# teamtomo/torch-motion-correction

Hardware: NVIDIA B200
Metric: movies_per_second_estimate_plus_correct (higher is better)
Workload: dtype f32

## Files before the change

torch_motion_correction_b200/csrc/optimizer_tiled.cu:

```cuda
#include "common.cuh"
#include <math.h>

namespace {

constexpr int kTileKy = 8, kTileKx = 16, kTileBins = kTileKy * kTileKx;
#ifndef TMC_CHUNK_FRAMES
#define TMC_CHUNK_FRAMES 8
#endif
constexpr int kChunkFrames = TMC_CHUNK_FRAMES;
constexpr int kMaxChunks = 256 / kChunkFrames;
constexpr int kTileThreads = 256;
constexpr int kCoefThreads = 1024;

struct StepParams {
  const float* spec;
  const int* tiles;
  int n_tiles, G, T;
  int ny, nx, KY, KX, ky_start;
  float inv_ny, inv_nx;
  const double* sum_norms;
  const float* eval_base;
  const float* w_t;
  const float* w_sp;
  int nt, nhw;
  const float* patch_scale;
  float pixel_spacing;
  int loss_type;
  float* coef;
  float* exp_avg;
  float* exp_avg_sq;
  float step_size, bc2_sqrt, w1, w2, b2, epsf, weight_decay;
  double* loss_out;
  float* grad_out;
  float* shifts;
  float* grad_shifts;
  double* q;
};

__device__ __forceinline__ uint32_t smem_u32(const void* p) { return (uint32_t)__cvta_generic_to_shared(p); }
__device__ __forceinline__ void mbar_init(uint64_t* bar, int count) {
  asm volatile("mbarrier.init.shared::cta.b64 [%0], %1;" ::"r"(smem_u32(bar)), "r"(count));
}
__device__ __forceinline__ void mbar_expect_tx(uint64_t* bar, uint32_t bytes) {
  asm volatile("mbarrier.arrive.expect_tx.shared::cta.b64 _, [%0], %1;" ::"r"(smem_u32(bar)), "r"(bytes) : "memory");
}
__device__ __forceinline__ void bulk_load(void* dst, const void* src, uint32_t bytes, uint64_t* bar) {
  asm volatile("cp.async.bulk.shared::cluster.global.mbarrier::complete_tx::bytes [%0], [%1], %2, [%3];" ::"r"(smem_u32(dst)),
               "l"(src), "r"(bytes), "r"(smem_u32(bar))
               : "memory");
}
__device__ __forceinline__ void mbar_wait_addr(uint32_t bar_addr, uint32_t parity) {
  asm volatile(
      "{\n"
      ".reg .pred P1;\n"
      "LAB_WAIT:\n"
      "mbarrier.try_wait.parity.shared::cta.b64 P1, [%0], %1;\n"
      "@P1 bra DONE;\n"
      "bra LAB_WAIT;\n"
      "DONE:\n"
      "}" ::"r"(bar_addr),
      "r"(parity)
      : "memory");
}
__device__ __forceinline__ void mbar_wait(uint64_t* bar, uint32_t parity) {
  asm volatile(
      "{\n"
      ".reg .pred P1;\n"
      "LAB_WAIT:\n"
      "mbarrier.try_wait.parity.shared::cta.b64 P1, [%0], %1;\n"
      "@P1 bra DONE;\n"
      "bra LAB_WAIT;\n"
      "DONE:\n"
      "}" ::"r"(smem_u32(bar)),
      "r"(parity)
      : "memory");
}

__device__ __forceinline__ float2 fast_cis(float x) {
  const float k = rintf(x * 0.15915494309189535f);
  float r = fmaf(k, -6.2831854820251465f, x);
  r = fmaf(k, 1.7484555e-7f, r);
  return make_float2(__cosf(r), __sinf(r));
}

__global__ void __launch_bounds__(kCoefThreads) local_coefficient_kernel(const StepParams p, int flags) {
  extern __shared__ float csm[];
  __shared__ double red[kCoefThreads / 32];
  const int tid = threadIdx.x;
  const int G = p.G, T = p.T, nt = p.nt, nhw = p.nhw;
  const int ncoef = 2 * nt * nhw, ngt = 2 * G * T;
  float* gs_s = csm;
  float* eb_s = gs_s + ngt;
  float* wt_s = eb_s + ngt;
  float* wsp_s = wt_s + T * nt;
  float* coef_s = wsp_s + G * nhw;
  float* u_s = coef_s + ncoef;
  float* ea_s = u_s + G * 2 * nt;
  float* eas_s = ea_s + ncoef;
  asm volatile("griddepcontrol.launch_dependents;");
  const float neg_inv_px = -1.0f / p.pixel_spacing;
  if (flags & 4)
    for (int i = tid; i < ngt; i += kCoefThreads) eb_s[i] = __ldg(p.eval_base + i);
  for (int i = tid; i < T * nt; i += kCoefThreads) wt_s[i] = __ldg(p.w_t + i);
  for (int i = tid; i < G * nhw; i += kCoefThreads) wsp_s[i] = __ldg(p.w_sp + i);
  asm volatile("griddepcontrol.wait;" ::: "memory");
  if (flags & 1)
    for (int i = tid; i < ngt; i += kCoefThreads) gs_s[i] = p.grad_shifts[i] * neg_inv_px;
  for (int i = tid; i < ncoef; i += kCoefThreads) coef_s[i] = p.coef[i];
  if (flags & (2 | 8))
    for (int i = tid; i < ncoef; i += kCoefThreads) {
      ea_s[i] = p.exp_avg[i];
      eas_s[i] = p.exp_avg_sq[i];
    }
  double l = 0.0;
  if (flags & 1) {
    for (int g = tid; g < G; g += kCoefThreads) {
      const double sc = (double)p.patch_scale[g];
      if (sc != 0.0) {
        const double sumA = p.sum_norms[g], qg = p.q[g];
        if (p.loss_type == 0) {
          const double a = (double)T / (double)(T - 1);
          l += sc * a * a * (sumA - qg / T);
        } else {
          l += -sc * (qg - sumA) / ((double)p.ny * (double)p.nx * (double)(T - 1));
        }
      }
    }
    l = warp_sum(l);
    if ((tid & 31) == 0) red[tid >> 5] = l;
  }
  __syncthreads();
  if (flags & 1) {
    if (tid == 0) {
      double s = 0.0;
      for (int i = 0; i < kCoefThreads / 32; ++i) s += red[i];
      *p.loss_out = s;
    }
    for (int i = tid; i < ngt; i += kCoefThreads) p.grad_shifts[i] = 0.f;
    for (int i = tid; i < G; i += kCoefThreads) p.q[i] = 0.0;
    for (int o = tid; o < G * 2 * nt; o += kCoefThreads) {
      const int k = o % nt, c = (o / nt) & 1, g = o / (2 * nt);
      float acc = 0.f;
      for (int t = 0; t < T; ++t) acc = fmaf(wt_s[t * nt + k], gs_s[(g * T + t) * 2 + c], acc);
      u_s[o] = acc;
    }
    __syncthreads();
    const float step_size = p.step_size, bc2_sqrt = p.bc2_sqrt, w1 = p.w1, w2 = p.w2, b2 = p.b2, epsf = p.epsf;
    for (int o = tid; o < ncoef; o += kCoefThreads) {
      const int j = o % nhw, ck = o / nhw;
      float acc = 0.f;
      for (int g = 0; g < G; ++g) acc = fmaf(wsp_s[g * nhw + j], u_s[g * 2 * nt + ck], acc);
      p.grad_out[o] = acc;
      if (flags & 2) {
        float gr = acc;
        float par = coef_s[o];
        if (p.weight_decay != 0.f) gr = __fadd_rn(gr, __fmul_rn(p.weight_decay, par));
        const float m = __fadd_rn(ea_s[o], __fmul_rn(w1, __fsub_rn(gr, ea_s[o])));
        const float v = __fadd_rn(__fmul_rn(eas_s[o], b2), __fmul_rn(w2, __fmul_rn(gr, gr)));
        p.exp_avg[o] = m;
        p.exp_avg_sq[o] = v;
        const float denom = __fadd_rn(__fdiv_rn(__fsqrt_rn(v), bc2_sqrt), epsf);
        par = __fadd_rn(par, __fmul_rn(-step_size, __fdiv_rn(m, denom)));
        p.coef[o] = par;
        coef_s[o] = par;
      }
    }
    __syncthreads();
  }
  if (flags & 8) {
    const float step_size = p.step_size, bc2_sqrt = p.bc2_sqrt, w1 = p.w1, w2 = p.w2, b2 = p.b2, epsf = p.epsf;
    for (int o = tid; o < ncoef; o += kCoefThreads) {
      float gr = p.grad_out[o];
      float par = coef_s[o];
      if (p.weight_decay != 0.f) gr = __fadd_rn(gr, __fmul_rn(p.weight_decay, par));
      const float m = __fadd_rn(ea_s[o], __fmul_rn(w1, __fsub_rn(gr, ea_s[o])));
      const float v = __fadd_rn(__fmul_rn(eas_s[o], b2), __fmul_rn(w2, __fmul_rn(gr, gr)));
      p.exp_avg[o] = m;
      p.exp_avg_sq[o] = v;
      const float denom = __fadd_rn(__fdiv_rn(__fsqrt_rn(v), bc2_sqrt), epsf);
      par = __fadd_rn(par, __fmul_rn(-step_size, __fdiv_rn(m, denom)));
      p.coef[o] = par;
      coef_s[o] = par;
    }
    __syncthreads();
  }
  if (!(flags & 4)) return;
  for (int o = tid; o < G * 2 * nt; o += kCoefThreads) {
    const int ck = o % (2 * nt), g = o / (2 * nt);
    float acc = 0.f;
    for (int j = 0; j < nhw; ++j) acc = fmaf(wsp_s[g * nhw + j], coef_s[ck * nhw + j], acc);
    u_s[o] = acc;
  }
  __syncthreads();
  for (int i = tid; i < ngt; i += kCoefThreads) {
    const int c = i & 1, t = (i >> 1) % T, g = (i >> 1) / T;
    float ev = 0.f;
    for (int k = 0; k < nt; ++k) ev = fmaf(wt_s[t * nt + k], u_s[(g * 2 + c) * nt + k], ev);
    const float v = __fmul_rn(-1.0f, __fadd_rn(ev, eb_s[(t * G + g) * 2 + c]));
    p.shifts[i] = __fdiv_rn(v, p.pixel_spacing);
  }
}

__global__ void __launch_bounds__(kTileThreads) local_loss_tile_kernel(const StepParams p) {
  constexpr int THREADS = kTileThreads;
  constexpr int NW = THREADS / 64;
  extern __shared__ __align__(128) unsigned char smem_raw[];
  const int T = p.T;
  float* tile = reinterpret_cast<float*>(smem_raw);
  float4* Ey = reinterpret_cast<float4*>(tile + (long)T * 256);
  float4* Ex = Ey + T * 8;
  float4* Cy = Ex + T * 8;
  float4* Cx = Cy + 64;
  float* sigma = reinterpret_cast<float*>(Cx + 64);
  float* cf = sigma + 256;
  double* red = reinterpret_cast<double*>(cf + 24);
  uint64_t* bars = reinterpret_cast<uint64_t*>(red + 2);

  const int tid = threadIdx.x;
  const int g = blockIdx.y, tile_id = blockIdx.x;
  const int nchunks = (T + kChunkFrames - 1) / kChunkFrames;
  asm volatile("griddepcontrol.launch_dependents;");

  if (tid == 0) {
    for (int c = 0; c < nchunks; ++c) mbar_init(bars + c, 1);
    asm volatile("fence.mbarrier_init.release.cluster;" ::: "memory");
    asm volatile("fence.proxy.async.shared::cta;" ::: "memory");
    const float* src = p.spec + ((long)g * p.n_tiles + tile_id) * T * 256;
    for (int c = 0; c < nchunks; ++c) {
      const int frames = min(kChunkFrames, T - c * kChunkFrames);
      const uint32_t bytes = (uint32_t)frames * 256 * sizeof(float);
      mbar_expect_tx(bars + c, bytes);
      bulk_load(tile + (long)c * kChunkFrames * 256, src + (long)c * kChunkFrames * 256, bytes, bars + c);
    }
  }
  const float sc = __ldg(p.patch_scale + g);
  const int ty = __ldg(p.tiles + 2 * tile_id), tx = __ldg(p.tiles + 2 * tile_id + 1);
  constexpr int kRowThreads = 96;
  const int my_r = tid < kRowThreads ? (tid & 7) : kTileKy + ((tid - kRowThreads) & 15);
  float my_cf;
  {
    if (my_r < kTileKy) {
      int ky = p.ky_start + min(ty * kTileKy + my_r, p.KY - 1);
      if (ky >= (p.ny + 1) / 2) ky -= p.ny;
      if (ky < -(p.ny / 2)) ky += p.ny;
      my_cf = __fmul_rn(-6.283185307179586f, __fmul_rn((float)ky, p.inv_ny));
    } else {
      my_cf = __fmul_rn(-6.283185307179586f, __fmul_rn((float)min(tx * kTileKx + my_r - kTileKy, p.KX - 1), p.inv_nx));
    }
    if (tid < kTileKy) cf[tid] = my_cf;
    if (tid >= kRowThreads && tid < kRowThreads + kTileKx) cf[kTileKy + tid - kRowThreads] = my_cf;
  }
  sigma[tid] = 0.f;
  asm volatile("griddepcontrol.wait;" ::: "memory");
  if (sc == 0.f || T < 2) {
    __syncthreads();
    for (int c = 0; c < nchunks; ++c) mbar_wait(bars + c, 0);
    return;
  }
  const float* shg = p.shifts + (long)g * T * 2;
  if (tid < kRowThreads) {
    for (int t = tid >> 3; t < T; t += kRowThreads / 8) {
      const float2 e = fast_cis(__fmul_rn(my_cf, shg[2 * t]));
      Ey[t * 8 + my_r] = make_float4(e.x, e.x, e.y, e.y);
    }
  } else {
    const int j = (tid - kRowThreads) & 15;
    for (int t = (tid - kRowThreads) >> 4; t < T; t += (kTileThreads - kRowThreads) / 16) {
      const float2 e = fast_cis(__fmul_rn(my_cf, shg[2 * t + 1]));
      float* o = reinterpret_cast<float*>(Ex + t * 8 + (j >> 1)) + (j & 1);
      o[0] = e.x;
      o[2] = e.y;
    }
  }
  __syncthreads();

  {
    const int pb = tid & 63, th = tid >> 6;
    const float4* ey = Ey + (pb >> 3) + th * 8;
    const float4* ex = Ex + (pb & 7) + th * 8;
    float2* col = reinterpret_cast<float2*>(tile) + pb + th * 128;
    float2 sre = make_float2(0.f, 0.f), sim = make_float2(0.f, 0.f);
    auto body = [&](const float4* eyp, const float4* exp_, float2* cp) {
      const float4 y = *eyp, x = *exp_;
      const float2 cy = make_float2(y.x, y.y), sy = make_float2(y.z, y.w);
      const float2 cx = make_float2(x.x, x.y), sx = make_float2(x.z, x.w);
      const float2 ere = __ffma2_rn(make_float2(-sy.x, -sy.y), sx, __fmul2_rn(cy, cx));
      const float2 eim = __ffma2_rn(sy, cx, __fmul2_rn(cy, sx));
      const float2 a = cp[0], b = cp[64];
      const float2 re = __ffma2_rn(make_float2(-b.x, -b.y), eim, __fmul2_rn(a, ere));
      const float2 im = __ffma2_rn(b, ere, __fmul2_rn(a, eim));
      cp[0] = re;
      cp[64] = im;
      sre = __fadd2_rn(sre, re);
      sim = __fadd2_rn(sim, im);
    };
    const uint32_t bar0 = smem_u32(bars);
    for (int c = 0; c < nchunks; ++c) {
      mbar_wait_addr(bar0 + 8u * c, 0);
      if ((c + 1) * kChunkFrames <= T) {
#pragma unroll
        for (int i = 0; i < kChunkFrames / NW; ++i) body(ey + i * NW * 8, ex + i * NW * 8, col + i * NW * 128);
      } else {
        for (int t = c * kChunkFrames + th, i = 0; t < T; t += NW, ++i) body(ey + i * NW * 8, ex + i * NW * 8, col + i * NW * 128);
      }
      ey += kChunkFrames * 8;
      ex += kChunkFrames * 8;
      col += kChunkFrames * 128;
    }
    atomicAdd(sigma + pb, sre.x);
    atomicAdd(sigma + 64 + pb, sre.y);
    atomicAdd(sigma + 128 + pb, sim.x);
    atomicAdd(sigma + 192 + pb, sim.y);
  }
  __syncthreads();
  if (tid < 64) {
    const int pb = tid;
    const float2 re = make_float2(sigma[pb], sigma[64 + pb]), im = make_float2(sigma[128 + pb], sigma[192 + pb]);
    const int kx0 = tx * kTileKx + 2 * (pb & 7);
    const float w0 = (p.loss_type == 0 || kx0 == 0 || 2 * kx0 == p.nx) ? 1.0f : 2.0f;
    const float w1 = (p.loss_type == 0 || 2 * (kx0 + 1) == p.nx) ? 1.0f : 2.0f;
    const float cfy = cf[pb >> 3], cfx0 = cf[8 + 2 * (pb & 7)], cfx1 = cf[9 + 2 * (pb & 7)];
    const float wr0 = w0 * re.x, wr1 = w1 * re.y, wi0 = w0 * im.x, wi1 = w1 * im.y;
    Cy[pb] = make_float4(cfy * wr0, cfy * wr1, -cfy * wi0, -cfy * wi1);
    Cx[pb] = make_float4(cfx0 * wr0, cfx1 * wr1, -cfx0 * wi0, -cfx1 * wi1);
  }
  __syncthreads();

  float bscale;
  if (p.loss_type == 0) {
    const float a = (float)T / (float)(T - 1);
    bscale = -sc * a * a / (float)T;
  } else {
    bscale = -sc / ((float)p.ny * (float)p.nx * (float)(T - 1));
  }
  const int lane = tid & 31, warp = tid >> 5;
  const int half = lane >> 4, l16 = lane & 15;
  for (int pi = warp; 2 * pi < T; pi += THREADS / 32) {
    const int t = 2 * pi + half;
    const bool ok = t < T;
    const float2* row = reinterpret_cast<const float2*>(tile + (long)(ok ? t : 0) * 256) + l16;
    float2 ay = make_float2(0.f, 0.f), ax = make_float2(0.f, 0.f);
#pragma unroll
    for (int k = 0; k < 4; ++k) {
      const float2 re = row[16 * k], im = row[64 + 16 * k];
      const float4 cy = Cy[l16 + 16 * k], cx = Cx[l16 + 16 * k];
      ay = __ffma2_rn(im, make_float2(cy.x, cy.y), ay);
      ay = __ffma2_rn(re, make_float2(cy.z, cy.w), ay);
      ax = __ffma2_rn(im, make_float2(cx.x, cx.y), ax);
      ax = __ffma2_rn(re, make_float2(cx.z, cx.w), ax);
    }
    const float gy = ay.x + ay.y, gx = ax.x + ax.y;
    const bool keep_x = (l16 & 8) != 0;
    float v = (keep_x ? gx : gy) + __shfl_xor_sync(0xffffffffu, keep_x ? gy : gx, 8);
#pragma unroll
    for (int o = 4; o > 0; o >>= 1) v += __shfl_xor_sync(0xffffffffu, v, o);
    if (ok && (l16 & 7) == 0) {
      v *= -2.0f * bscale;
      if (v != 0.f) atomicAdd(p.grad_shifts + ((long)g * T + t) * 2 + (keep_x ? 1 : 0), v);
    }
  }
  if (tid < 64) {
    const int pb = tid;
    const float2 re = make_float2(sigma[pb], sigma[64 + pb]), im = make_float2(sigma[128 + pb], sigma[192 + pb]);
    const int kx0 = tx * kTileKx + 2 * (pb & 7);
    const float w0 = (p.loss_type == 0 || kx0 == 0 || 2 * kx0 == p.nx) ? 1.0f : 2.0f;
    const float w1 = (p.loss_type == 0 || 2 * (kx0 + 1) == p.nx) ? 1.0f : 2.0f;
    double v = (double)w0 * ((double)re.x * re.x + (double)im.x * im.x) + (double)w1 * ((double)re.y * re.y + (double)im.y * im.y);
    v = warp_sum(v);
    if ((tid & 31) == 0 && v != 0.0) atomicAdd(p.q + g, v);
  }
}

__global__ void tile_spectra_kernel(const float2* __restrict__ spec, int T, int Tp, int KY, int KX, const int* __restrict__ tiles,
                                    int n_tiles, int frame_major, float* __restrict__ out) {
  const int tile_id = blockIdx.x, t = blockIdx.y, g = blockIdx.z, G = gridDim.z;
  const int b = threadIdx.x;
  const int kyb = tiles[2 * tile_id] * kTileKy + b / kTileKx, kx = tiles[2 * tile_id + 1] * kTileKx + b % kTileKx;
  float2 v = make_float2(0.f, 0.f);
  const long plane = frame_major ? ((long)(t >> 1) * G + g) * 2 + (t & 1) : (long)g * Tp + t;
  if (kyb < KY && kx < KX) v = spec[(plane * KY + kyb) * KX + kx];
  float* o = out + (((long)g * n_tiles + tile_id) * T + t) * 2 * kTileBins;
  o[b] = v.x;
  o[kTileBins + b] = v.y;
}

size_t tile_smem_bytes(int t) {
  return (size_t)t * kTileBins * 8 + (size_t)t * 16 * 16 + 128 * 16 + 256 * 4 + 24 * 4 + 2 * 8 +
         (size_t)((t + kChunkFrames - 1) / kChunkFrames) * 8;
}
size_t coef_smem_bytes(int g, int t, int nt, int nhw) {
  return ((size_t)4 * g * t + (size_t)t * nt + (size_t)g * nhw + (size_t)6 * nt * nhw + (size_t)g * 2 * nt) * 4;
}

}

TMC_API int tmc_local_steps_supported(int g, int t, int nt, int nhw) {
  if (t < 2 || t > kChunkFrames * kMaxChunks || g < 1 || g > 65535 || nt < 1 || nhw < 1) return 0;
  if (tile_smem_bytes(t) > 200 * 1024) return 0;
  return coef_smem_bytes(g, t, nt, nhw) <= 160 * 1024 ? 1 : 0;
}

TMC_API int tmc_local_tile_spectra(const void* spec, int g, int t, int tp, int ky_count, int kx_count, const int* tiles,
                                   int n_tiles, int frame_major, void* out, cudaStream_t stream) {
  TMC_CHECK_ARG(spec && tiles && out && g >= 1 && t >= 1 && tp >= t && n_tiles >= 1 && t <= 65535 && g <= 65535,
                "local_tile_spectra: bad arguments");
  dim3 grid(n_tiles, t, g);
  tile_spectra_kernel<<<grid, kTileBins, 0, stream>>>((const float2*)spec, t, tp, ky_count, kx_count, tiles, n_tiles, frame_major, (float*)out);
  tmc_count_launch();
  TMC_CHECK_LAUNCH("tmc_local_tile_spectra");
  return TMC_OK;
}

TMC_API long tmc_local_steps_workspace_bytes(int g, int t, int nt) {
  (void)nt;
  long floats = 4l * g * t;
  floats = (floats + 1) & ~1l;
  return floats * 4 + 8l * g;
}

TMC_API int tmc_local_steps(const void* tiled, const int* tiles, int n_tiles, int g, int t, int ny, int nx, int ky_count,
                            int kx_count, int ky_start, const double* sum_norms, const float* eval_base, const float* w_t,
                            const float* w_sp, int nt, int nhw, const float* patch_scale, float pixel_spacing, int loss_type,
                            float* coef, float* exp_avg, float* exp_avg_sq, double lr, double beta1, double beta2, double eps,
                            double weight_decay, int first_row, int mode, int n_steps, double* loss_out, float* grad_out,
                            void* workspace, cudaStream_t stream) {
  TMC_CHECK_ARG(tiled && tiles && sum_norms && eval_base && w_t && w_sp && patch_scale && coef && loss_out && grad_out && workspace,
                "local_steps: null pointer");
  TMC_CHECK_ARG(mode >= 0 && mode <= 3, "local_steps: mode must be 0 .. 3");
  TMC_CHECK_ARG(mode == 1 || (exp_avg && exp_avg_sq), "local_steps: Adam state missing");
  TMC_CHECK_ARG(mode == 0 || n_steps == 1, "local_steps: modes 1 .. 3 take one step");
  TMC_CHECK_ARG(n_tiles >= 1 && n_steps >= 1 && first_row >= 0 && pixel_spacing > 0.f && (loss_type == 0 || loss_type == 1),
                "local_steps: bad arguments");
  if (!tmc_local_steps_supported(g, t, nt, nhw)) {
    tmc_set_error("local_steps: unsupported problem size (g=%d t=%d nt=%d nhw=%d)", g, t, nt, nhw);
    return TMC_ERR_UNSUPPORTED;
  }
  StepParams p;
  p.spec = (const float*)tiled;
  p.tiles = tiles;
  p.n_tiles = n_tiles;
  p.G = g;
  p.T = t;
  p.ny = ny;
  p.nx = nx;
  p.KY = ky_count;
  p.KX = kx_count;
  p.ky_start = ky_start;
  p.inv_ny = (float)(1.0 / (double)ny);
  p.inv_nx = (float)(1.0 / (double)nx);
  p.sum_norms = sum_norms;
  p.eval_base = eval_base;
  p.w_t = w_t;
  p.w_sp = w_sp;
  p.nt = nt;
  p.nhw = nhw;
  p.pixel_spacing = pixel_spacing;
  p.loss_type = loss_type;
  p.coef = coef;
  p.exp_avg = exp_avg;
  p.exp_avg_sq = exp_avg_sq;
  p.w1 = (float)(1.0 - beta1);
  p.w2 = (float)(1.0 - beta2);
  p.b2 = (float)beta2;
  p.epsf = (float)eps;
  p.weight_decay = (float)weight_decay;
  p.step_size = 0.f;
  p.bc2_sqrt = 1.f;
  p.grad_out = grad_out;
  float* wf = (float*)workspace;
  p.shifts = wf;
  p.grad_shifts = wf + 2l * g * t;
  const long floats = (4l * g * t + 1) & ~1l;
  p.q = (double*)(wf + floats);
  if (mode < 2) TMC_CUDA(cudaMemsetAsync(workspace, 0, (size_t)tmc_local_steps_workspace_bytes(g, t, nt), stream));
  const size_t smem = tile_smem_bytes(t), csmem = coef_smem_bytes(g, t, nt, nhw);
  TMC_CUDA(cudaFuncSetAttribute(local_loss_tile_kernel, cudaFuncAttributeMaxDynamicSharedMemorySize, (int)(200 * 1024)));
  TMC_CUDA(cudaFuncSetAttribute(local_coefficient_kernel, cudaFuncAttributeMaxDynamicSharedMemorySize, (int)(160 * 1024)));
  dim3 grid(n_tiles, g);
  p.patch_scale = patch_scale + (long)first_row * g;
  p.loss_out = loss_out;
  if (mode >= 2) {
    const double step = (double)first_row;
    p.step_size = (float)(lr / (1.0 - pow(beta1, step)));
    p.bc2_sqrt = (float)sqrt(1.0 - pow(beta2, step));
  }
  local_coefficient_kernel<<<1, kCoefThreads, csmem, stream>>>(p, mode == 2 ? (8 | 4) : (mode == 3 ? 8 : 4));
  tmc_count_launch();
  if (mode == 3) {
    TMC_CHECK_LAUNCH("tmc_local_steps");
    return TMC_OK;
  }
  cudaLaunchAttribute attr[1];
  attr[0].id = cudaLaunchAttributeProgrammaticStreamSerialization;
  attr[0].val.programmaticStreamSerializationAllowed = 1;
  cudaLaunchConfig_t cfg = {};
  cfg.gridDim = grid;
  cfg.blockDim = dim3(kTileThreads);
  cfg.dynamicSmemBytes = smem;
  cfg.stream = stream;
  cfg.attrs = attr;
  cfg.numAttrs = 1;
  cudaLaunchConfig_t ccfg = {};
  ccfg.gridDim = dim3(1);
  ccfg.blockDim = dim3(kCoefThreads);
  ccfg.dynamicSmemBytes = csmem;
  ccfg.stream = stream;
  ccfg.attrs = attr;
  ccfg.numAttrs = 1;
  for (int i = 0; i < n_steps; ++i) {
    const int row = first_row + i;
    p.patch_scale = patch_scale + (long)row * g;
    const double step = (double)(row + 1);
    p.step_size = (float)(lr / (1.0 - pow(beta1, step)));
    p.bc2_sqrt = (float)sqrt(1.0 - pow(beta2, step));
    p.loss_out = loss_out + (mode == 0 ? row : 0);
    TMC_CUDA(cudaLaunchKernelEx(&cfg, local_loss_tile_kernel, p));
    tmc_count_launch();
    const int last = i == n_steps - 1;
    TMC_CUDA(cudaLaunchKernelEx(&ccfg, local_coefficient_kernel, p, mode == 0 ? (last ? 3 : 7) : 1));
    tmc_count_launch();
  }
  TMC_CHECK_LAUNCH("tmc_local_steps");
  return TMC_OK;
}
```

Baseline: 51.65.

## Add persistent register-resident tiled loss kernel with double-buffered bulk loads

Adds a templated loss kernel for short frame counts (up to 64) that keeps each tile's spectra in registers, runs as a persistent grid sized to the occupancy limit, and double-buffers tile loads with TMA bulk copies and mbarriers. Per-frame gradient sums use a shuffle transpose-reduce instead of shared-memory reductions, and the arithmetic uses packed float2 math. The old shared-memory kernel stays as the fallback for larger T. Risks are higher register pressure and lower occupancy.

```diff
diff --git a/torch_motion_correction_b200/csrc/optimizer_tiled.cu b/torch_motion_correction_b200/csrc/optimizer_tiled.cu
--- a/torch_motion_correction_b200/csrc/optimizer_tiled.cu
+++ b/torch_motion_correction_b200/csrc/optimizer_tiled.cu
@@ -1,5 +1,7 @@
 #include "common.cuh"
 #include <math.h>
+
+#include <algorithm>
 
 namespace {
 
@@ -11,6 +13,8 @@
 constexpr int kMaxChunks = 256 / kChunkFrames;
 constexpr int kTileThreads = 256;
 constexpr int kCoefThreads = 1024;
+constexpr int kRegWarps = kTileThreads / 32;
+constexpr int kRegMaxFrames = 8;
 
 struct StepParams {
   const float* spec;
@@ -98,6 +102,9 @@
   float* ea_s = u_s + G * 2 * nt;
   float* eas_s = ea_s + ncoef;
   asm volatile("griddepcontrol.launch_dependents;");
+#ifdef TMC_COEF_NOOP
+  return;
+#endif
   const float neg_inv_px = -1.0f / p.pixel_spacing;
   if (flags & 4)
     for (int i = tid; i < ngt; i += kCoefThreads) eb_s[i] = __ldg(p.eval_base + i);
@@ -201,7 +208,243 @@
   }
 }
 
+__device__ __forceinline__ float tile_freq(const StepParams& p, int ty, int tx, int r) {
+  if (r < kTileKy) {
+    int ky = p.ky_start + min(ty * kTileKy + r, p.KY - 1);
+    if (ky >= (p.ny + 1) / 2) ky -= p.ny;
+    if (ky < -(p.ny / 2)) ky += p.ny;
+    return __fmul_rn(-6.283185307179586f, __fmul_rn((float)ky, p.inv_ny));
+  }
+  return __fmul_rn(-6.283185307179586f, __fmul_rn((float)min(tx * kTileKx + r - kTileKy, p.KX - 1), p.inv_nx));
+}
+
+template <int N, int O>
+__device__ __forceinline__ float transpose_reduce(const float (&v)[N], int lane, int& idx, int& live) {
+  if constexpr (N == 1) {
+    float s = v[0];
+#pragma unroll
+    for (int o = O; o > 0; o >>= 1) s += __shfl_xor_sync(0xffffffffu, s, o);
+    if (O > 0 && (lane & (2 * O - 1)) != 0) live = 0;
+    return s;
+  } else {
+    static_assert(O > 0, "more values than lanes");
+    constexpr int H = (N + 1) / 2;
+    const bool up = (lane & O) != 0;
+    float w[H];
+#pragma unroll
+    for (int i = 0; i < H; ++i) {
+      const float lo = v[i], hi = i + H < N ? v[i + H] : 0.f;
+      w[i] = (up ? hi : lo) + __shfl_xor_sync(0xffffffffu, up ? lo : hi, O);
+    }
+    if (up) {
+      idx += H;
+      live -= H;
+    } else {
+      live = min(live, H);
+    }
+    return transpose_reduce<H, O / 2>(w, lane, idx, live);
+  }
+}
+
+template <int NF>
 __global__ void __launch_bounds__(kTileThreads) local_loss_tile_kernel(const StepParams p) {
+  constexpr int TF = NF * kRegWarps;
+  extern __shared__ __align__(128) float4 ring[];
+  __shared__ float2 ey_s[TF][kTileKy];
+  __shared__ float4 exc_s[TF][kTileKx / 4];
+  __shared__ float4 exs_s[TF][kTileKx / 4];
+  __shared__ float4 part_s[kRegWarps][2][32];
+  __shared__ __align__(16) float sig_s[2 * kTileBins];
+  __shared__ __align__(16) float cf_s[kTileKy + kTileKx];
+  __shared__ uint64_t bars[2];
+
+  const int tid = threadIdx.x, lane = tid & 31, warp = tid >> 5;
+  const int T = p.T, nblk = p.n_tiles * p.G;
+  const int nk = (nblk - (int)blockIdx.x + (int)gridDim.x - 1) / (int)gridDim.x;
+  const uint32_t tile_bytes = (uint32_t)T * 2 * kTileBins * sizeof(float);
+  auto block_of = [&](int k) { return (int)blockIdx.x + k * (int)gridDim.x; };
+  auto issue = [&](int k) {
+    mbar_expect_tx(bars + (k & 1), tile_bytes);
+    bulk_load(ring + (long)(k & 1) * T * 64, p.spec + (long)block_of(k) * T * 2 * kTileBins, tile_bytes, bars + (k & 1));
+  };
+  asm volatile("griddepcontrol.launch_dependents;");
+#ifdef TMC_LOSS_WAIT_ONLY
+  asm volatile("griddepcontrol.wait;" ::: "memory");
+  return;
+#endif
+  if (tid == 0) {
+    mbar_init(bars, 1);
+    mbar_init(bars + 1, 1);
+    asm volatile("fence.mbarrier_init.release.cluster;" ::: "memory");
+    asm volatile("fence.proxy.async.shared::cta;" ::: "memory");
+    for (int k = 0; k < min(2, nk); ++k) issue(k);
+  }
+  __syncthreads();
+  asm volatile("griddepcontrol.wait;" ::: "memory");
+  constexpr int kSlots = kTileKy + kTileKx, kSweep = kTileThreads / kSlots;
+  constexpr int kSlotFrames = (TF + kSweep - 1) / kSweep;
+  const int slot = tid % kSlots;
+  const int row = lane >> 2, cq = lane & 3;
+  float sc_next = 0.f, sh_next[kSlotFrames];
+  int ty_next = 0, tx_next = 0;
+  auto fetch = [&](int k) {
+    const int blk = block_of(k), g = blk / p.n_tiles, tile_id = blk - g * p.n_tiles;
+    sc_next = __ldg(p.patch_scale + g);
+    ty_next = __ldg(p.tiles + 2 * tile_id);
+    tx_next = __ldg(p.tiles + 2 * tile_id + 1);
+    const float* shg = p.shifts + (long)g * T * 2 + (slot < kTileKy ? 0 : 1);
+#pragma unroll
+    for (int j = 0; j < kSlotFrames; ++j) {
+      const int t = tid / kSlots + j * kSweep;
+      sh_next[j] = tid < kSweep * kSlots && t < T ? shg[2 * t] : 0.f;
+    }
+  };
+  if (nk > 0) fetch(0);
+
+  for (int k = 0; k < nk; ++k) {
+    const int blk = block_of(k), g = blk / p.n_tiles;
+    const float sc = sc_next;
+    const int ty = ty_next, tx = tx_next;
+    float sh[kSlotFrames];
+#pragma unroll
+    for (int j = 0; j < kSlotFrames; ++j) sh[j] = sh_next[j];
+    if (k + 1 < nk) fetch(k + 1);
+    mbar_wait(bars + (k & 1), (k >> 1) & 1);
+    float4 fre[NF], fim[NF];
+    {
+      const float4* src = ring + (long)(k & 1) * T * 64 + lane;
+#pragma unroll
+      for (int i = 0; i < NF; ++i) {
+        const int t = warp + kRegWarps * i;
+        if (t < T) {
+          fre[i] = src[t * 64];
+          fim[i] = src[t * 64 + 32];
+        } else {
+          fre[i] = fim[i] = make_float4(0.f, 0.f, 0.f, 0.f);
+        }
+      }
+    }
+    __syncthreads();
+    if (tid == 0 && k + 2 < nk) {
+      asm volatile("fence.proxy.async.shared::cta;" ::: "memory");
+      issue(k + 2);
+    }
+    if (sc == 0.f) continue;
+    {
+      const float slot_cf = tile_freq(p, ty, tx, slot);
+      if (tid < kSlots) cf_s[tid] = slot_cf;
+#pragma unroll
+      for (int j = 0; j < kSlotFrames; ++j) {
+        const int t = tid / kSlots + j * kSweep;
+        if (tid < kSweep * kSlots && t < T) {
+          const float2 e = fast_cis(__fmul_rn(slot_cf, sh[j]));
+          if (slot < kTileKy) {
+            ey_s[t][slot] = e;
+          } else {
+            reinterpret_cast<float*>(exc_s[t])[slot - kTileKy] = e.x;
+            reinterpret_cast<float*>(exs_s[t])[slot - kTileKy] = e.y;
+          }
+        }
+      }
+    }
+    __syncthreads();
+
+    float2 s0re = make_float2(0.f, 0.f), s0im = s0re, s1re = s0re, s1im = s0re;
+#pragma unroll
+    for (int i = 0; i < NF; ++i) {
+      const int t = warp + kRegWarps * i;
+      if (t < T) {
+        const float2 y = ey_s[t][row];
+        const float4 xc = exc_s[t][cq], xs = exs_s[t][cq];
+        const float2 cy = make_float2(y.x, y.x), sy = make_float2(y.y, y.y), nsy = make_float2(-y.y, -y.y);
+        auto rot = [&](float2 cx, float2 sx, float2 a, float2 b, float2& re, float2& im) {
+          const float2 ere = __ffma2_rn(nsy, sx, __fmul2_rn(cy, cx));
+          const float2 eim = __ffma2_rn(sy, cx, __fmul2_rn(cy, sx));
+          re = __ffma2_rn(make_float2(-b.x, -b.y), eim, __fmul2_rn(a, ere));
+          im = __ffma2_rn(b, ere, __fmul2_rn(a, eim));
+        };
+        float2 r0, i0, r1, i1;
+        rot(make_float2(xc.x, xc.y), make_float2(xs.x, xs.y), make_float2(fre[i].x, fre[i].y), make_float2(fim[i].x, fim[i].y), r0, i0);
+        rot(make_float2(xc.z, xc.w), make_float2(xs.z, xs.w), make_float2(fre[i].z, fre[i].w), make_float2(fim[i].z, fim[i].w), r1, i1);
+        fre[i] = make_float4(r0.x, r0.y, r1.x, r1.y);
+        fim[i] = make_float4(i0.x, i0.y, i1.x, i1.y);
+        s0re = __fadd2_rn(s0re, r0);
+        s0im = __fadd2_rn(s0im, i0);
+        s1re = __fadd2_rn(s1re, r1);
+        s1im = __fadd2_rn(s1im, i1);
+      }
+    }
+    part_s[warp][0][lane] = make_float4(s0re.x, s0re.y, s1re.x, s1re.y);
+    part_s[warp][1][lane] = make_float4(s0im.x, s0im.y, s1im.x, s1im.y);
+    __syncthreads();
+    {
+      const float* pf = reinterpret_cast<const float*>(part_s);
+      float s = 0.f;
+#pragma unroll
+      for (int w = 0; w < kRegWarps; ++w) s += pf[w * 2 * kTileBins + tid];
+      sig_s[tid] = s;
+    }
+    __syncthreads();
+
+    const float4 sre = reinterpret_cast<const float4*>(sig_s)[lane], sim = reinterpret_cast<const float4*>(sig_s)[32 + lane];
+    const int kx0 = tx * kTileKx + 4 * cq;
+    const float wgt[4] = {(p.loss_type == 0 || kx0 == 0 || 2 * kx0 == p.nx) ? 1.0f : 2.0f,
+                          (p.loss_type == 0 || 2 * (kx0 + 1) == p.nx) ? 1.0f : 2.0f,
+                          (p.loss_type == 0 || 2 * (kx0 + 2) == p.nx) ? 1.0f : 2.0f,
+                          (p.loss_type == 0 || 2 * (kx0 + 3) == p.nx) ? 1.0f : 2.0f};
+    const float wr[4] = {wgt[0] * sre.x, wgt[1] * sre.y, wgt[2] * sre.z, wgt[3] * sre.w};
+    const float wi[4] = {wgt[0] * sim.x, wgt[1] * sim.y, wgt[2] * sim.z, wgt[3] * sim.w};
+    {
+      const float cfy = cf_s[row];
+      const float4 cx4 = reinterpret_cast<const float4*>(cf_s)[kTileKy / 4 + cq];
+      const float cfx[4] = {cx4.x, cx4.y, cx4.z, cx4.w};
+      const float2 cyr0 = make_float2(cfy * wr[0], cfy * wr[1]), cyr1 = make_float2(cfy * wr[2], cfy * wr[3]);
+      const float2 cyi0 = make_float2(-cfy * wi[0], -cfy * wi[1]), cyi1 = make_float2(-cfy * wi[2], -cfy * wi[3]);
+      const float2 cxr0 = make_float2(cfx[0] * wr[0], cfx[1] * wr[1]), cxr1 = make_float2(cfx[2] * wr[2], cfx[3] * wr[3]);
+      const float2 cxi0 = make_float2(-cfx[0] * wi[0], -cfx[1] * wi[1]), cxi1 = make_float2(-cfx[2] * wi[2], -cfx[3] * wi[3]);
+      float v[2 * NF];
+#pragma unroll
+      for (int i = 0; i < NF; ++i) {
+        const float2 re0 = make_float2(fre[i].x, fre[i].y), re1 = make_float2(fre[i].z, fre[i].w);
+        const float2 im0 = make_float2(fim[i].x, fim[i].y), im1 = make_float2(fim[i].z, fim[i].w);
+        float2 ay = __ffma2_rn(im0, cyr0, make_float2(0.f, 0.f)), ax = __ffma2_rn(im0, cxr0, make_float2(0.f, 0.f));
+        ay = __ffma2_rn(re0, cyi0, ay);
+        ax = __ffma2_rn(re0, cxi0, ax);
+        ay = __ffma2_rn(im1, cyr1, ay);
+        ax = __ffma2_rn(im1, cxr1, ax);
+        ay = __ffma2_rn(re1, cyi1, ay);
+        ax = __ffma2_rn(re1, cxi1, ax);
+        v[2 * i] = ay.x + ay.y;
+        v[2 * i + 1] = ax.x + ax.y;
+      }
+      int idx = 0, live = 2 * NF;
+      float s = transpose_reduce<2 * NF, 16>(v, lane, idx, live);
+      const int t = warp + kRegWarps * (idx >> 1);
+      if (live > 0 && t < T) {
+        float bscale;
+        if (p.loss_type == 0) {
+          const float a = (float)T / (float)(T - 1);
+          bscale = -sc * a * a / (float)T;
+        } else {
+          bscale = -sc / ((float)p.ny * (float)p.nx * (float)(T - 1));
+        }
+        s *= -2.0f * bscale;
+        if (s != 0.f) atomicAdd(p.grad_shifts + ((long)g * T + t) * 2 + (idx & 1), s);
+      }
+    }
+    if (warp == 0) {
+      double q = 0.0;
+      q += (double)wgt[0] * ((double)sre.x * sre.x + (double)sim.x * sim.x);
+      q += (double)wgt[1] * ((double)sre.y * sre.y + (double)sim.y * sim.y);
+      q += (double)wgt[2] * ((double)sre.z * sre.z + (double)sim.z * sim.z);
+      q += (double)wgt[3] * ((double)sre.w * sre.w + (double)sim.w * sim.w);
+      q = warp_sum(q);
+      if (lane == 0 && q != 0.0) atomicAdd(p.q + g, q);
+    }
+  }
+}
+
+__global__ void __launch_bounds__(kTileThreads) local_loss_tile_smem_kernel(const StepParams p) {
   constexpr int THREADS = kTileThreads;
   constexpr int NW = THREADS / 64;
   extern __shared__ __align__(128) unsigned char smem_raw[];
@@ -382,6 +625,22 @@
   float* o = out + (((long)g * n_tiles + tile_id) * T + t) * 2 * kTileBins;
   o[b] = v.x;
   o[kTileBins + b] = v.y;
+}
+
+using LossKernel = void (*)(StepParams);
+LossKernel register_loss_kernel(int t) {
+  static_assert(kRegMaxFrames == 8, "one case per frame count");
+  switch ((t + kRegWarps - 1) / kRegWarps) {
+    case 1: return local_loss_tile_kernel<1>;
+    case 2: return local_loss_tile_kernel<2>;
+    case 3: return local_loss_tile_kernel<3>;
+    case 4: return local_loss_tile_kernel<4>;
+    case 5: return local_loss_tile_kernel<5>;
+    case 6: return local_loss_tile_kernel<6>;
+    case 7: return local_loss_tile_kernel<7>;
+    case 8: return local_loss_tile_kernel<8>;
+    default: return nullptr;
+  }
 }
 
 size_t tile_smem_bytes(int t) {
@@ -473,10 +732,25 @@
   const long floats = (4l * g * t + 1) & ~1l;
   p.q = (double*)(wf + floats);
   if (mode < 2) TMC_CUDA(cudaMemsetAsync(workspace, 0, (size_t)tmc_local_steps_workspace_bytes(g, t, nt), stream));
-  const size_t smem = tile_smem_bytes(t), csmem = coef_smem_bytes(g, t, nt, nhw);
-  TMC_CUDA(cudaFuncSetAttribute(local_loss_tile_kernel, cudaFuncAttributeMaxDynamicSharedMemorySize, (int)(200 * 1024)));
+  LossKernel loss_kernel = register_loss_kernel(t);
+  size_t smem;
+  dim3 grid(n_tiles, g);
+  if (loss_kernel) {
+    smem = (size_t)2 * t * kTileBins * 8;
+  } else {
+    loss_kernel = local_loss_tile_smem_kernel;
+    smem = tile_smem_bytes(t);
+  }
+  const size_t csmem = coef_smem_bytes(g, t, nt, nhw);
+  TMC_CUDA(cudaFuncSetAttribute(loss_kernel, cudaFuncAttributeMaxDynamicSharedMemorySize, (int)(200 * 1024)));
   TMC_CUDA(cudaFuncSetAttribute(local_coefficient_kernel, cudaFuncAttributeMaxDynamicSharedMemorySize, (int)(160 * 1024)));
-  dim3 grid(n_tiles, g);
+  if (loss_kernel != local_loss_tile_smem_kernel) {
+    int dev = 0, sms = 0, per_sm = 0;
+    TMC_CUDA(cudaGetDevice(&dev));
+    TMC_CUDA(cudaDeviceGetAttribute(&sms, cudaDevAttrMultiProcessorCount, dev));
+    TMC_CUDA(cudaOccupancyMaxActiveBlocksPerMultiprocessor(&per_sm, loss_kernel, kTileThreads, smem));
+    grid = dim3((unsigned)std::min<long>((long)n_tiles * g, (long)std::max(per_sm, 1) * sms));
+  }
   p.patch_scale = patch_scale + (long)first_row * g;
   p.loss_out = loss_out;
   if (mode >= 2) {
@@ -514,7 +788,7 @@
     p.step_size = (float)(lr / (1.0 - pow(beta1, step)));
     p.bc2_sqrt = (float)sqrt(1.0 - pow(beta2, step));
     p.loss_out = loss_out + (mode == 0 ? row : 0);
-    TMC_CUDA(cudaLaunchKernelEx(&cfg, local_loss_tile_kernel, p));
+    TMC_CUDA(cudaLaunchKernelEx(&cfg, loss_kernel, p));
     tmc_count_launch();
     const int last = i == n_steps - 1;
     TMC_CUDA(cudaLaunchKernelEx(&ccfg, local_coefficient_kernel, p, mode == 0 ? (last ? 3 : 7) : 1));
```

Measured after the change: 52.75, median of 6. 1.02x the previous value.
